# PlantandFoodResearch/MCHap

Hardware: AMD Instinct MI355X
Metric: loci/sec (whole node) for 1000-step MCMC, tetraploid 8-SNV loci, 1/2/4/8 GPUs (higher is better)
Workload: dtype f64; 1 GPU; 10000 synthetic tetraploid loci per GPU, 8 SNVs, 200 reads, 1000 MCMC steps x 2 chains, burn 500, posterior summary (BASELINE.json configs[1]); 4 passes in flight on separate HIP streams, each with its own device buffers; loci_per_gpu=10000, ploidy=4, snvs=8, reads=200, mcmc_steps=1000, chains=2, burn=500, llk_cache=True, passes_in_flight=4, hw_queues=4, world_size=1, devices=1

## Files before the change

### mchap_amd/csrc/denovo_simt_kernel.hpp

```cpp
#pragma once
#include "denovo_kernel.hpp"

namespace mchap {

constexpr int META_I_MH = 0;
constexpr int META_I_STATUS = 1;
constexpr int META_I_NDICT = 2;
constexpr int META_I_FLAT = 3;
constexpr int META_I_W01 = 4;
constexpr int META_I_COLS = 5;
__host__ __device__ inline int meta_i_stride(int max_pos) { return 5 + 2 * max_pos; }
constexpr uint16_t ND_W01 = 0x8000u;
__host__ __device__ inline int nd_count(uint16_t x) { return (int)(x & 0x7FFFu); }
__host__ __device__ inline bool nd_w01(uint16_t x) { return (x & ND_W01) != 0; }
constexpr int DICT_MAX = 128;
constexpr int DICT_HASH = 512;
__host__ __device__ inline int meta_f_prior(int) { return 1; }
__host__ __device__ inline int meta_f_dist(int max_ploidy) { return 1 + 2 * max_ploidy + 5; }
__host__ __device__ inline int meta_f_stride(int max_ploidy, int max_pos, int max_allele) {
  return 1 + 2 * max_ploidy + 5 + max_pos * max_allele;
}

struct SimtParams {
  DenovoParams d;
  double *rt;
  double *cntw;
  uint8_t *codes;
  double *dict;
  double *gbp;
  int32_t *meta_i;
  double *meta_f;
  int n_units;
  int max_pos, max_allele, max_ploidy;
  int max_ma;
  int max_ugens_pad;
  int prep_rows_off;
  int cstride;
  int flags;
  void *lane_state;
  void *lane_memo;
  void *pipe_state;
  double *pipe_memo;
  const int32_t *pipe_list;
  const int32_t *pipe_count;
  int32_t *pipe_out;
  int32_t *pipe_out_count;
  int pipe_iters;
  int pipe_iters_max;
  int pipe_mode;
  int pipe_parts;
  int bp_cache;
  int fill_lt, fill_kw;
  int tw_lds;
  int word_bits;
  uint64_t cache_epoch;
  uint64_t *ctx;
  int ctx_n;
};
constexpr int PIPE_RESUME = 1;
constexpr int PIPE_EXPORT = 2;
constexpr int PIPE_FILLONLY = 4;
constexpr int PIPE_NOFILL = 8;
constexpr int PIPE_FILL_SLOTS = 1024;
__host__ __device__ inline int pipe_parts_eff(int n_list, int parts) {
  if (parts <= 1 || n_list <= 0) return 1;
  const int pe = PIPE_FILL_SLOTS / n_list;
  return pe < 1 ? 1 : (pe > parts ? parts : pe);
}
struct PipeState {
  uint64_t g[8];
  double llk;
  uint64_t ctr;
  double mlo, mhi;
  int32_t step;
  int32_t mvalid;
  uint64_t pad[3];
};
static_assert(sizeof(PipeState) == 128, "PipeState layout");
constexpr int SIMT_FLAG_PREP_GLOBAL = 1 << 30;

#ifndef MCHAP_PREP_WPE
#define MCHAP_PREP_WPE 4
#endif
template <int RPL>
__global__ __launch_bounds__(64, MCHAP_PREP_WPE) void denovo_prepare_kernel(const SimtParams P) {
  extern __shared__ __align__(16) unsigned char smem[];
  const DenovoParams &D = P.d;
  const int u = blockIdx.x;
  const mchap_unit U = D.units[u];
  const int lane = threadIdx.x;
  const int R = U.n_reads, M0 = U.n_pos, A = U.max_allele, K = U.ploidy;
  const int rpad = D.rpad;
  const int MA = M0 * A;
  double *rt = P.rt + (size_t)u * P.max_ma * rpad;
  const bool in_lds = !(P.flags & SIMT_FLAG_PREP_GLOBAL);
  double *rl = in_lds ? reinterpret_cast<double *>(smem) : rt;
  double *lp = reinterpret_cast<double *>(smem) + (in_lds ? (size_t)MA * rpad : 0);
  const double *gr = D.reads ? D.reads + U.reads_off : nullptr;
  const int8_t *nal0 = D.n_alleles + U.nalleles_off;
  auto rawv = [&](int r, int q) -> double {
    if (gr) return gr[(size_t)r * MA + q];
    const int j = q / A, a = q - j * A;
    if (a >= nal0[j]) return 0.0;
    const size_t e = (size_t)U.reads_off + (size_t)r * M0 + j;
    const int call = D.calls[e];
    if (call < 0) return NAN;
    int qi = D.quals ? (int)D.quals[e] : 0;
    qi = qi < 0 ? 0 : (qi >= D.qual_prob_len ? D.qual_prob_len - 1 : qi);
    const double pc = D.qual_prob[qi];
    return a == call ? pc : (1.0 - pc) / 3.0;
  };
  double *cw = P.cntw + (size_t)u * rpad;
  int32_t *mi = P.meta_i + (size_t)u * meta_i_stride(P.max_pos);
  double *mf = P.meta_f + (size_t)u * meta_f_stride(P.max_ploidy, P.max_pos, P.max_allele);

  bool all_gaps = true;
  for (int r = lane; r < rpad; r += WAVE) {
    for (int q0 = 0; q0 < MA; q0 += 8) {
      double v[8];
#pragma unroll
      for (int k = 0; k < 8; k++) v[k] = (r < R && q0 + k < MA) ? rawv(r, q0 + k) : 1.0;
#pragma unroll
      for (int k = 0; k < 8; k++) {
        const int q = q0 + k;
        if (q < MA) {
          const double x = isnan(v[k]) ? 1.0 : v[k];
          if (in_lds) rl[(size_t)q * rpad + r] = x;
          rt[(size_t)q * rpad + r] = x;
          if (q % A < (int)nal0[q / A]) all_gaps = all_gaps && (x == 1.0);
        }
      }
    }
  }
  {
    const bool flat = __ballot(!all_gaps) == 0ull;
    if (lane == 0) mi[META_I_FLAT] = flat ? 1 : 0;
  }
  double cnt[RPL];
#pragma unroll
  for (int i = 0; i < RPL; i++) {
    const int r = lane + WAVE * i;
    cnt[i] = (r < R) ? (U.counts_off >= 0 ? (double)D.counts[U.counts_off + r] : 1.0) : 0.0;
    cw[r] = cnt[i];
  }
  {
    bool w01 = true;
#pragma unroll
    for (int i = 0; i < RPL; i++) w01 = w01 && (cnt[i] == 0.0 || cnt[i] == 1.0);
    const bool all01 = __ballot(!w01) == 0ull;
    if (lane == 0) mi[META_I_W01] = (all01 && !(P.flags & (1 << 20))) ? 1 : 0;
  }
  __syncthreads();
  {
    unsigned long long *hkeys = reinterpret_cast<unsigned long long *>(lp + P.max_ugens_pad);
    uint16_t *hcode = reinterpret_cast<uint16_t *>(hkeys + DICT_HASH);
    int *ndist = reinterpret_cast<int *>(hcode + DICT_HASH);
    const unsigned long long EMPTY = ~0ull;
    for (int i = lane; i < DICT_HASH; i += WAVE) hkeys[i] = EMPTY;
    if (lane == 0) *ndist = 0;
    __syncthreads();
    const int RPLT = rpad / WAVE;
    for (int q = 0; q < MA; q++) {
      for (int i0 = 0; i0 < RPL; i0 += 4) {
      unsigned long long keys[4];
#pragma unroll
      for (int k = 0; k < 4; k++) keys[k] = (unsigned long long)__double_as_longlong(rt[(size_t)q * rpad + lane + WAVE * min(i0 + k, RPL - 1)]);
#pragma unroll
      for (int k = 0; k < 4; k++) {
        if (i0 + k >= RPL) break;
        const unsigned long long key = keys[k];
        unsigned slot = (unsigned)(mix64(key) & (DICT_HASH - 1));
        while (*(volatile int *)ndist <= DICT_MAX) {
          unsigned long long old = *(volatile unsigned long long *)&hkeys[slot];
          if (old == EMPTY) {
            old = atomicCAS(&hkeys[slot], EMPTY, key);
            if (old == EMPTY) atomicAdd(ndist, 1);
          }
          if (old == EMPTY || old == key) break;
          slot = (slot + 1) & (DICT_HASH - 1);
        }
      }
      }
    }
    __syncthreads();
    const int nd = *ndist;
    uint8_t *ct = P.codes + (size_t)u * P.max_ma * WAVE * P.cstride;
    double *dict = P.dict + (size_t)u * DICT_MAX;
    if (nd <= DICT_MAX) {
      int base = 0;
      for (int s0 = 0; s0 < DICT_HASH; s0 += WAVE) {
        const unsigned long long key = hkeys[s0 + lane];
        const bool occ = key != EMPTY;
        const unsigned long long m = __ballot(occ);
        const int code = base + __popcll(m & ((1ull << lane) - 1ull));
        if (occ) {
          hcode[s0 + lane] = (uint16_t)code;
          dict[code] = __longlong_as_double((long long)key);
        }
        base += __popcll(m);
      }
      __syncthreads();
      for (int q = 0; q < MA; q++) {
        for (int i0 = 0; i0 < RPL; i0 += 4) {
          unsigned long long keys[4];
#pragma unroll
          for (int k = 0; k < 4; k++) keys[k] = (unsigned long long)__double_as_longlong(rt[(size_t)q * rpad + lane + WAVE * min(i0 + k, RPL - 1)]);
          uint32_t packed = 0;
#pragma unroll
          for (int k = 0; k < 4; k++) {
            if (i0 + k >= RPL) break;
            const unsigned long long key = keys[k];
            unsigned slot = (unsigned)(mix64(key) & (DICT_HASH - 1));
            while (hkeys[slot] != key) slot = (slot + 1) & (DICT_HASH - 1);
            if (RPL > 2) packed |= (uint32_t)(uint8_t)hcode[slot] << (8 * k);
            else ct[((size_t)q * WAVE + lane) * P.cstride + i0 + k] = (uint8_t)hcode[slot];
          }
          if (RPL > 2) *reinterpret_cast<uint32_t *>(ct + ((size_t)q * WAVE + lane) * P.cstride + i0) = packed;
        }
      }
    }
    if (lane == 0) mi[META_I_NDICT] = nd <= DICT_MAX ? nd : 0;
  }
  const int8_t *nalleles = D.n_alleles + U.nalleles_off;
  int Mh = 0;
  double luh = 0.0;
  const bool pow2_ploidy = (K & (K - 1)) == 0;
  const double inv_ploidy = 1.0 / (double)K;
  constexpr int KP = MCHAP_MAX_PLOIDY_DENOVO;
  __shared__ double s_lg1[KP + 1];
  __shared__ double s_lga[(MCHAP_MAX_ALLELE + 1) * (KP + 1)];
  __shared__ double s_lgb[MCHAP_MAX_ALLELE + 1], s_left[MCHAP_MAX_ALLELE + 1];
  const double Fp = U.inbreeding;
  const bool with_prior = !isnan(Fp);
  if (with_prior) {
    for (int d = lane; d <= K; d += WAVE) s_lg1[d] = lgamma((double)d + 1.0);
    if (Fp != 0.0) {
      for (int e = lane; e < (A + 1) * (K + 1); e += WAVE) {
        const int n = e / (K + 1), d = e % (K + 1);
        if (n >= 1 && d >= 1) s_lga[n * (KP + 1) + d] = lgamma((double)d + (1.0 / (double)n) * ((1.0 - Fp) / Fp));
      }
      for (int n = 1 + lane; n <= A; n += WAVE) {
        const double alpha = (1.0 / (double)n) * ((1.0 - Fp) / Fp);
        const double sum_alphas = alpha * (double)n;
        s_lgb[n] = lgamma(alpha);
        s_left[n] = (lgamma((double)K + 1.0) + lgamma(sum_alphas)) - lgamma((double)K + sum_alphas);
      }
    }
    __syncthreads();
  }
  auto snv_prior = [&](uint64_t g, int n) -> double {
    int dose[KP];
    for (int i = 0; i < K; i++) dose[i] = 0;
    for (int i = 0; i < K; i++) {
      int j = 0;
      while (nib(g, i) != nib(g, j)) j++;
      dose[j] += 1;
    }
    if (Fp == 0.0) {
      double den = 0.0;
      for (int i = 0; i < K; i++) den += s_lg1[dose[i]];
      return (s_lg1[K] - den) - (double)K * c_ln[n];
    }
    double prod = 0.0;
    for (int i = 0; i < K; i++)
      if (dose[i] > 0) prod += s_lga[n * (KP + 1) + dose[i]] - (s_lg1[dose[i]] + s_lgb[n]);
    return s_left[n] + prod;
  };
  double *pl = reinterpret_cast<double *>(smem + P.prep_rows_off);
  for (int j = 0; j < M0; j++) {
    const int n = nalleles[j];
    const int u_gens = snv_genotypes(n, K);
    const double *rowp = rl + (size_t)(j * A) * rpad;
    if (!in_lds) {
      for (int a = 0; a < A; a++)
#pragma unroll
        for (int i = 0; i < RPL; i++) pl[(size_t)a * rpad + lane + WAVE * i] = rt[(size_t)(j * A + a) * rpad + lane + WAVE * i];
      rowp = pl;
    }
    uint64_t g = 0;
    for (int q = 0; q < u_gens; q++) {
      double lprior = 0.0;
      if (with_prior) lprior = snv_prior(g, n);
      double s = 0.0;
#pragma unroll
      for (int i = 0; i < RPL; i++) {
        double rp = 0.0;
        if (pow2_ploidy) {
          for (int h = 0; h < K; h++) rp += rowp[(size_t)nib(g, h) * rpad + lane + WAVE * i] * inv_ploidy;
        } else {
          for (int h = 0; h < K; h++) rp += rowp[(size_t)nib(g, h) * rpad + lane + WAVE * i] / (double)K;
        }
        s += read_log(rp) * cnt[i];
      }
      const double llk = wave_sum(s);
      lp[q] = lprior + llk;
      g = increment_snv_genotype(g, K);
    }
    double acc = lp[0];
    for (int q = 1; q < u_gens; q++) acc = add_log_prob(acc, lp[q]);
    int fixed_allele = -1;
    for (int a = 0; a < n; a++) {
      int idx = 0;
      for (int i = 0; i < K; i++) idx += (a == 0) ? 0 : snv_genotypes(a, i + 1);
      if (exp(lp[idx] - acc) >= D.fix_hom) fixed_allele = a;
    }
    if (lane == 0) D.fixed[U.fixed_off + j] = (int8_t)fixed_allele;
    if (fixed_allele < 0) {
      if (lane == 0) {
        mi[META_I_COLS + Mh] = j * A;
        mi[META_I_COLS + P.max_pos + Mh] = n;
      }
      luh += c_ln[n];
      Mh++;
    }
  }
  const int bits = allele_bits(A);
  int status = MCHAP_UNIT_OK;
  if (Mh == 0) status = MCHAP_UNIT_ALL_FIXED;
  else if (Mh * bits > (P.word_bits ? P.word_bits : 64)) status = MCHAP_ERR_LIMIT;
  else if (U.initial_off >= 0 && U.initial_n_het != Mh) status = MCHAP_UNIT_BAD_INITIAL;
  if (lane == 0) {
    mi[META_I_MH] = Mh;
    mi[META_I_STATUS] = status;
    D.status[u] = status;
    mf[0] = luh;
  }
  if (status != MCHAP_UNIT_OK) {
    if (status == MCHAP_UNIT_ALL_FIXED) {
      const size_t tb = U.trace_off, lb = U.llk_off;
      const int S = D.steps, C_ = D.chains;
      for (int i = lane; i < C_ * S * K; i += WAVE) D.trace[tb + i] = 0ull;
      for (int i = lane; i < C_ * S; i += WAVE) D.llks[lb + i] = NAN;
    }
    return;
  }
  if (!isnan(U.inbreeding) && lane == 0) {
    double *t = mf + meta_f_prior(0);
    const double F = U.inbreeding;
    for (int d = 0; d <= K; d++) t[K + 1 + d] = lgamma((double)d + 1.0);
    t[2 * K + 3] = lgamma((double)K + 1.0);
    t[2 * K + 4] = (double)K * luh;
    if (F != 0.0) {
      const double log_disp = log((1.0 - F) / F) - luh;
      const double disp = exp(log_disp);
      const double sum_disp = exp(log_disp + luh);
      const double lg_disp = lgamma(disp);
      t[0] = 0.0;
      for (int d = 1; d <= K; d++) t[d] = lgamma((double)d + disp) - (lgamma((double)d + 1.0) + lg_disp);
      t[2 * K + 2] = (lgamma((double)K + 1.0) + lgamma(sum_disp)) - lgamma((double)K + sum_disp);
    }
  }
  if (U.initial_off < 0) {
    double *dist = mf + meta_f_dist(P.max_ploidy);
    __syncthreads();
    for (int jj = 0; jj < Mh; jj++) {
      const int col = mi[META_I_COLS + jj];
      int n_nonzero = 0;
      uint32_t gapmask = 0;
      double dv[MCHAP_MAX_ALLELE];
      for (int a = 0; a < A; a++) {
        double tot = 0.0;
        int n_ok = 0, n_nz = 0;
        for (int i0 = 0; i0 < RPL; i0 += 4) {
          double v4[4];
#pragma unroll
          for (int k = 0; k < 4; k++) {
            const int r = lane + WAVE * (i0 + k);
            v4[k] = (i0 + k < RPL && r < R) ? rawv(r, col + a) : 0.0;
          }
#pragma unroll
          for (int k = 0; k < 4; k++) {
            const int r = lane + WAVE * (i0 + k);
            if (i0 + k < RPL && r < R) {
              const double v = v4[k];
              if (!isnan(v)) {
                tot += v;
                n_ok++;
              }
              if (!(v == 0.0)) n_nz++;
            }
          }
        }
        tot = wave_sum(tot);
        n_ok = wave_sum_i(n_ok);
        n_nz = wave_sum_i(n_nz);
        if (n_ok == 0) {
          gapmask |= 1u << a;
          dv[a] = 1.0;
          n_nonzero++;
        } else {
          dv[a] = tot / (double)n_ok;
          if (n_nz > 0) n_nonzero++;
        }
      }
      for (int a = 0; a < A; a++)
        if (gapmask & (1u << a)) dv[a] = 1.0 / (double)n_nonzero;
      double s = 0.0;
      for (int a = 1; a < A; a++) s += dv[a];
      s = (A > 1) ? dv[0] + s : dv[0];
      if (lane == 0)
        for (int a = 0; a < A; a++) dist[jj * A + a] = dv[a] / s;
    }
  }
}

typedef unsigned __int128 u128;
template <class W> struct WordBits { static constexpr int value = 8 * (int)sizeof(W); };
__device__ __forceinline__ int word_popc(uint64_t x) { return __popcll(x); }
__device__ __forceinline__ int word_popc(u128 x) { return __popcll((uint64_t)x) + __popcll((uint64_t)(x >> 64)); }
__device__ __forceinline__ int word_ffs(uint64_t x) { return __ffsll((long long)x); }
__device__ __forceinline__ int word_ffs(u128 x) {
  const uint64_t lo = (uint64_t)x, hi = (uint64_t)(x >> 64);
  return lo ? __ffsll((long long)lo) : (hi ? 64 + __ffsll((long long)hi) : 0);
}
__device__ __forceinline__ uint64_t word_mix(uint64_t t, uint64_t x) { return mix64(t ^ x) + 0x9E3779B97F4A7C15ull; }
__device__ __forceinline__ uint64_t word_mix(uint64_t t, u128 x) {
  t = mix64(t ^ (uint64_t)(x >> 64)) + 0x9E3779B97F4A7C15ull;
  return mix64(t ^ (uint64_t)x) + 0x9E3779B97F4A7C15ull;
}

template <class W> struct PackOf { typedef uint32_t type; static constexpr int KMAX = MCHAP_MAX_PLOIDY; };
template <> struct PackOf<u128> { typedef uint64_t type; static constexpr int KMAX = MCHAP_MAX_PLOIDY_DENOVO; };

template <class W>
struct SimtLdsT {
  W *w;
  W *pw;
  double *llk_t;
  uint64_t *rngn;
  double *prior;
  uint8_t *optin;
  uint16_t *sub;
  uint16_t *cols;
  uint8_t *shift;
  uint8_t *nal;
};
typedef SimtLdsT<uint64_t> SimtLds;

__host__ __device__ inline size_t simt_lds_bytes(int Kmax, int Mmax, int T, int word_bytes = 8) {
  size_t b = 0;
  b += (size_t)word_bytes * T * Kmax * 64;
  b += (size_t)word_bytes * Kmax * 64;
  b += (size_t)8 * T * 64 * 2;
  b += (size_t)8 * (2 * Kmax + 5) * 64;
  b += (size_t)Kmax * Kmax * 64;
  b += (size_t)2 * Kmax * Mmax * 64;
  b += (size_t)2 * Mmax * 64;
  b += (size_t)1 * Mmax * 64 * 2;
  return (b + 15) & ~(size_t)15;
}

// ... 737 lines not shown
```

### mchap_amd/csrc/mchap_hip.hip

```cpp
#include <hip/hip_runtime.h>

#include <cmath>
#include <cstdarg>
#include <cstdio>
#include <cstdlib>
#include <cstring>
#include <algorithm>
#include <atomic>
#include <mutex>
#include <vector>

#include "../../include/mchap_hip.h"
#include "denovo_kernel.hpp"
#include "denovo_simt_kernel.hpp"
#include "denovo_spec_kernel.hpp"
#include "denovo_fillw_kernel.hpp"
#ifdef MCHAP_TEST_KERNELS
#include "denovo_fill_kernel.hpp"
#include "denovo_lane_kernel.hpp"
#endif
#include "exact_kernel.hpp"
#include "call_mcmc_kernel.hpp"
#include "posterior_kernel.hpp"

// ... 182 lines not shown
}

struct DevBuf {
  void *p = nullptr;
  ~DevBuf() {
    if (p) (void)hipFree(p);
  }
  template <class T>
  T *as() const { return reinterpret_cast<T *>(p); }
};

struct HostCall {
  hipStream_t stream = nullptr;
  int open() {
    HIP_TRY(hipStreamCreateWithFlags(&stream, hipStreamNonBlocking));
    return MCHAP_OK;
  }
  ~HostCall() {
    if (stream) (void)hipStreamDestroy(stream);
  }
  int up(void *dst, const void *src, size_t bytes) {
    HIP_TRY(hipMemcpyAsync(dst, src, bytes, hipMemcpyHostToDevice, stream));
    return MCHAP_OK;
  }
  int down(void *dst, const void *src, size_t bytes) {
    HIP_TRY(hipMemcpyAsync(dst, src, bytes, hipMemcpyDeviceToHost, stream));
    return MCHAP_OK;
  }
  int sync() {
    HIP_TRY(hipStreamSynchronize(stream));
    return MCHAP_OK;
  }
};
#define MCHAP_TRY(expr)       \
  do {                        \
    const int rc_ = (expr);   \
    if (rc_) return rc_;      \
  } while (0)

size_t up256(size_t x) { return (x + 255) & ~(size_t)255; }
struct DevArena {
  DevBuf buf;
  size_t cap = 0, off = 0;
  int reserve(size_t bytes) {
    cap = bytes + 4096;
    if (hipMalloc(&buf.p, cap) != hipSuccess) return fail(MCHAP_ERR_HIP, "hipMalloc of %zu bytes", cap);
    return MCHAP_OK;
  }
  template <class T>
  T *take(size_t n) {
    T *p = reinterpret_cast<T *>(reinterpret_cast<unsigned char *>(buf.p) + off);
    off += up256(n * sizeof(T));
    return off <= cap ? p : nullptr;
  }
};

int code_stride(int rpl) { return rpl <= 2 ? rpl : (rpl + 3) & ~3; }

int rpl_for(int max_reads) {
  const int need = (max_reads + 63) / 64;
  for (int r : {1, 2, 4, 8, 16})
    if (need <= r) return r;
  return -1;
}

int validate_cfg(const mchap_denovo_cfg *cfg) {
  if (!cfg) return fail(MCHAP_ERR_BAD_ARG, "cfg is NULL");
  if (cfg->steps < 1 || cfg->chains < 1) return fail(MCHAP_ERR_BAD_ARG, "steps and chains must be >= 1");
  if (cfg->chains > 65535) return fail(MCHAP_ERR_LIMIT, "chains > 65535");
  if (cfg->n_temps < 1 || cfg->n_temps > MCHAP_MAX_TEMPS) return fail(MCHAP_ERR_LIMIT, "n_temps out of range");
  for (int t = 1; t < cfg->n_temps; t++)
    if (cfg->temperatures[t] < cfg->temperatures[t - 1]) return fail(MCHAP_ERR_BAD_ARG, "temperatures must be ascending");
  if (cfg->temperatures[0] < 0.0) return fail(MCHAP_ERR_BAD_ARG, "temperatures must be >= 0");
  if (cfg->temperatures[cfg->n_temps - 1] != 1.0) return fail(MCHAP_ERR_BAD_ARG, "last temperature must be 1.0");
  if (cfg->n_intervals == 0 && !cfg->break_table) return fail(MCHAP_ERR_BAD_ARG, "break_table required when n_intervals is None");
#ifndef MCHAP_TEST_KERNELS
  if (cfg->kernel == 1 || cfg->kernel == 4)
    return fail(MCHAP_ERR_BAD_ARG, "kernel %d is only built into libmchap_hip_test.so (make test-kernels)", cfg->kernel);
#endif
  if (cfg->kernel < 0 || cfg->kernel > 5) return fail(MCHAP_ERR_BAD_ARG, "kernel %d: not one of 0..5", cfg->kernel);
  return MCHAP_OK;
}

struct Tune {
  int cache_slots = 1024, flags = 0, spec_group = 0, pipe_first = 0, pipe_resume = 8, pipe_rounds = 2, pipe_max = 64, pipe_parts = 8;
  int pipe_group = 64;
  size_t prep_lds_limit = 8 * 1024;
  int pipe_stop = 0;
  bool cache_auto = true;
};
Tune tune_of(const mchap_denovo_cfg *cfg) {
  Tune t;
  const mchap_denovo_tuning *u = cfg->tuning;
  if (!u) return t;
  if (u->cache_slots >= 64 && u->cache_slots <= 65536 && (u->cache_slots & (u->cache_slots - 1)) == 0) {
    t.cache_slots = u->cache_slots;
    t.cache_auto = false;
  }
  t.flags = u->flags;
  if (u->spec_group == 16 || u->spec_group == 32 || u->spec_group == 64) t.spec_group = u->spec_group;
  if (u->pipe_first > 0) t.pipe_first = u->pipe_first;
  if (u->pipe_resume > 0) t.pipe_resume = u->pipe_resume;
  if (u->pipe_rounds > 0) t.pipe_rounds = u->pipe_rounds - 1;
  if (u->pipe_max > 0) t.pipe_max = u->pipe_max;
  if (u->pipe_parts > 0 && u->pipe_parts <= 64) t.pipe_parts = u->pipe_parts;
  if (u->prep_lds_limit > 0) t.prep_lds_limit = (size_t)u->prep_lds_limit;
  t.pipe_stop = u->pipe_stop;
#ifdef MCHAP_TEST_KERNELS
  if (u->reserved[0] == 16 || u->reserved[0] == 32) t.pipe_group = u->reserved[0];
#endif
  return t;
}

size_t break_table_bytes(const mchap_denovo_cfg *cfg) {
  const size_t mp = cfg->max_pos > 0 ? (size_t)cfg->max_pos : 1;
  return ((mp + 1) * mp * sizeof(double) + 255) & ~(size_t)255;
}

struct BatchDims {
  int max_reads = 1, max_pos = 1, max_allele = 1, max_ploidy = 1, max_ma = 1, max_ugens = 1;
  int min_reads = 1 << 30;
  int uniform_ploidy = -1;
};

bool use_simt(const mchap_denovo_cfg *cfg);
int batch_dims(const mchap_denovo_cfg *cfg, int n_units, const mchap_unit *units_host, BatchDims &B) {
  for (int u = 0; u < n_units; u++) {
    const mchap_unit &U = units_host[u];
    const int kmax = use_simt(cfg) ? MCHAP_MAX_PLOIDY_DENOVO : MCHAP_MAX_PLOIDY;
    if (U.ploidy < 1 || U.ploidy > kmax) return fail(MCHAP_ERR_LIMIT, "unit %d: ploidy %d not in 1..%d", u, U.ploidy, kmax);
    if (U.max_allele < 1 || U.max_allele > MCHAP_MAX_ALLELE) return fail(MCHAP_ERR_LIMIT, "unit %d: max_allele %d not in 1..%d", u, U.max_allele, MCHAP_MAX_ALLELE);
    if (U.n_reads < 1 || U.n_reads > MCHAP_MAX_READS) return fail(MCHAP_ERR_LIMIT, "unit %d: n_reads %d not in 1..%d (zero reads are mocked by the caller as one NaN read)", u, U.n_reads, MCHAP_MAX_READS);
    if (U.n_pos < 1 || U.n_pos > MCHAP_MAX_POS) return fail(MCHAP_ERR_LIMIT, "unit %d: n_pos %d not in 1..%d", u, U.n_pos, MCHAP_MAX_POS);
    if (cfg->n_intervals == 0 && U.n_pos > cfg->max_pos) return fail(MCHAP_ERR_BAD_ARG, "unit %d: n_pos exceeds break_table", u);
    B.max_reads = std::max(B.max_reads, U.n_reads);
    B.min_reads = std::min(B.min_reads, U.n_reads);
    B.max_pos = std::max(B.max_pos, U.n_pos);
    B.max_allele = std::max(B.max_allele, U.max_allele);
    B.max_ploidy = std::max(B.max_ploidy, U.ploidy);
    B.uniform_ploidy = (B.uniform_ploidy < 0 || B.uniform_ploidy == U.ploidy) ? U.ploidy : 0;
    B.max_ma = std::max(B.max_ma, U.n_pos * U.max_allele);
    B.max_ugens = std::max(B.max_ugens, mchap::snv_genotypes(U.max_allele, U.ploidy));
  }
  return MCHAP_OK;
}

int spec_group(const Tune &T, int K, int max_pos) {
  if (K < 2 || K > 8) return 0;
  const int n = K * max_pos;
  int g = T.spec_group ? T.spec_group : 16;
  while (g < 64 && (g < K * (K - 1) || 2 * g < n)) g *= 2;
  const int slots = (g == 64) ? 3 : 2;
  if (g < K * (K - 1) || slots * g < n) return 0;
  if ((K == 5 || K == 6) && g < 32) g = 32;
  if (K >= 7) g = 64;
  return g;
}

bool lane_supported(int K, int max_pos, int n_temps) {
#ifdef MCHAP_TEST_KERNELS
  if (n_temps != 1 || K < 1 || K > 8) return false;
  const int slots = (K == 8) ? 3 : 2;
  return K * max_pos <= slots * 64 && K * (K - 1) <= 64;
#else
  return false;
#endif
// ... 639 lines not shown
  P.seed = cfg->seed;
  P.rpad = rpad;
  P.max_pos = cfg->max_pos > 0 ? cfg->max_pos : 1;
  {
    const size_t n = (size_t)(P.max_pos + 1) * P.max_pos;
    const size_t bt_bytes = break_table_bytes(cfg);
    if (!workspace || workspace_bytes < (int64_t)bt_bytes)
      return fail(MCHAP_ERR_BAD_ARG, "workspace of %lld bytes is too small (mchap_denovo_workspace_bytes)", (long long)workspace_bytes);
    double *bt_dev = reinterpret_cast<double *>(workspace);
    if (cfg->break_table)
      HIP_TRY(hipMemcpyAsync(bt_dev, cfg->break_table, n * sizeof(double), hipMemcpyHostToDevice, stream));
    else
      HIP_TRY(hipMemsetAsync(bt_dev, 0, n * sizeof(double), stream));
    P.break_table = bt_dev;
    workspace = reinterpret_cast<unsigned char *>(workspace) + bt_bytes;
    workspace_bytes -= (int64_t)bt_bytes;
  }
  HIP_TRY(hipMemsetAsync(status, 0, sizeof(int32_t) * n_units, stream));
  P.cache = nullptr;
  P.cache_slots = 0;

  if (use_simt(cfg)) {
    const int want_slots = cache_slots_of(cfg, T, pl, n_units, B);
    int slots = want_slots;
    SimtCarve cv = simt_carve(cfg, pl, n_units, B, rpad, slots);
    while (slots >= 32 && (int64_t)cv.total > workspace_bytes) {
      slots >>= 1;
      cv = simt_carve(cfg, pl, n_units, B, rpad, slots);
    }
    if (slots < 32 && want_slots) {
      slots = 0;
      cv = simt_carve(cfg, pl, n_units, B, rpad, 0);
    }
    if (!workspace || (int64_t)cv.total > workspace_bytes)
      return fail(MCHAP_ERR_BAD_ARG, "workspace of %lld bytes is too small: kernel %d needs at least %zu (mchap_denovo_workspace_bytes)",
                  (long long)workspace_bytes, cfg->kernel, cv.total);
    unsigned char *ws = reinterpret_cast<unsigned char *>(workspace);
    if (ctx_shape(pl, B, T) && workspace_bytes > (int64_t)cv.total) {
      const int cn = ctx_slots_for((size_t)(workspace_bytes - (int64_t)cv.total), (size_t)n_units * cfg->chains, ctx_slot_bytes(pl, B));
      if (cn > 0) {
        SP.ctx = reinterpret_cast<uint64_t *>(ws + cv.ctx);
        SP.ctx_n = cn;
      }
    }
    if (slots > 0) {
      P.cache = reinterpret_cast<uint64_t *>(ws + cv.cache);
      P.cache_slots = slots;
      uint64_t epoch = 0;
      if ((pl.kind == SAMPLER_PIPE || pl.kind == SAMPLER_SPEC) && !(T.flags & (64 | 65536)) &&
          B.max_ploidy * mchap::allele_bits(B.max_allele) * B.max_pos <= 32) {
        epoch = cfg->cache_epoch > 0 ? (uint64_t)cfg->cache_epoch : g_cache_epoch.fetch_add(1) + 1;
        if (epoch >= (1ull << 31) - 1) epoch = 0;
      }
      SP.cache_epoch = epoch << 33;
      if (!epoch)
        HIP_TRY(hipMemsetAsync(ws + cv.cache, 0, (size_t)n_units * cfg->chains * (pl.kind == SAMPLER_SPEC ? cfg->n_temps : 1) * slots * 16, stream));
      if (cv.key_words) {
        P.cache_keys = reinterpret_cast<uint64_t *>(ws + cv.ckeys);
        P.cache_key_words = cv.key_words;
      }
    }
    SP.rt = reinterpret_cast<double *>(ws + cv.rt);
    SP.cntw = reinterpret_cast<double *>(ws + cv.cntw);
    SP.codes = ws + cv.codes;
    SP.dict = reinterpret_cast<double *>(ws + cv.dict);
    SP.gbp = (cv.has_gbp && !(T.flags & 512)) ? reinterpret_cast<double *>(ws + cv.gbp) : nullptr;
    SP.meta_i = reinterpret_cast<int32_t *>(ws + cv.meta_i);
    SP.meta_f = reinterpret_cast<double *>(ws + cv.meta_f);
    SP.lane_state = ws + cv.lane_state;
    SP.lane_memo = ws + cv.lane_memo;
    SP.pipe_state = ws + cv.pipe_state;
    SP.pipe_memo = reinterpret_cast<double *>(ws + cv.pipe_memo);
    SP.n_units = n_units;
    SP.max_pos = B.max_pos;
    SP.max_allele = B.max_allele;
    SP.max_ploidy = B.max_ploidy;
    SP.max_ma = B.max_ma;
    SP.cstride = code_stride(rpl);
    SP.flags = T.flags & (63 | 128 | 2048 | 4096 | 262144 | (1 << 20));
    SP.max_ugens_pad = (B.max_ugens + 8) & ~7;
    const size_t lds_dict = (size_t)mchap::DICT_HASH * (8 + 2) + 64;
    size_t lds_prep = (size_t)B.max_ma * rpad * 8 + (size_t)SP.max_ugens_pad * 8 + lds_dict;
    SP.prep_rows_off = 0;
    if (lds_prep > 160 * 1024 || (size_t)B.max_ma * rpad * 8 > T.prep_lds_limit) {
      lds_prep = (size_t)SP.max_ugens_pad * 8 + lds_dict;
      lds_prep = (lds_prep + 15) & ~(size_t)15;
      SP.prep_rows_off = (int)lds_prep;
      lds_prep += (size_t)B.max_allele * rpad * 8;
      SP.flags |= mchap::SIMT_FLAG_PREP_GLOBAL;
    }
    const size_t lds_simt = mchap::simt_lds_bytes(B.max_ploidy, B.max_pos, cfg->n_temps, pl.wide ? 16 : 8);
    SP.word_bits = pl.wide ? 128 : 64;
    if (lds_prep > 160 * 1024 || lds_simt > 160 * 1024)
      return fail(MCHAP_ERR_LIMIT, "a unit needs %zu / %zu bytes of LDS (> 160 KiB)", lds_prep, lds_simt);
    auto prepare = [&](const mchap::SimtParams &Q, int n, hipStream_t st) {
      switch (rpl) {
        case 1: return launch_prepare<1>(Q, n, lds_prep, st);
        case 2: return launch_prepare<2>(Q, n, lds_prep, st);
        case 3: return launch_prepare<3>(Q, n, lds_prep, st);
        case 4: return launch_prepare<4>(Q, n, lds_prep, st);
        case 5: return launch_prepare<5>(Q, n, lds_prep, st);
        case 6: return launch_prepare<6>(Q, n, lds_prep, st);
        case 7: return launch_prepare<7>(Q, n, lds_prep, st);
        case 8: return launch_prepare<8>(Q, n, lds_prep, st);
        case 12: return launch_prepare<12>(Q, n, lds_prep, st);
        case 16: return launch_prepare<16>(Q, n, lds_prep, st);
        case 24: return launch_prepare<24>(Q, n, lds_prep, st);
        case 32: return launch_prepare<32>(Q, n, lds_prep, st);
        case 48: return launch_prepare<48>(Q, n, lds_prep, st);
        default: return launch_prepare<64>(Q, n, lds_prep, st);
      }
    };
    rc = prepare(SP, n_units, stream);
    if (rc) return rc;
    switch (pl.kind) {
#ifdef MCHAP_TEST_KERNELS
      case SAMPLER_LANE: return launch_lane(T, pl.K, SP, n_units, cfg->chains, cfg->timer, stream);
#endif
      case SAMPLER_PIPE:
        return launch_pipe(T, pl.K, pl.G, SP, n_units, cfg->chains, reinterpret_cast<int32_t *>(ws + cv.pipe_lists),
                           reinterpret_cast<int32_t *>(ws + cv.pipe_counts), cfg->timer, stream, B.min_reads <= 64, B.max_reads);
      case SAMPLER_SPEC: return launch_spec(T, pl.K, pl.G, SP, n_units, cfg->chains, cfg->n_temps, cfg->timer, stream);
      default: return launch_simt(pl.K, SP, n_units, cfg->chains, lds_simt, cfg->timer, stream, pl.wide);
    }
  }

#ifdef MCHAP_TEST_KERNELS
  size_t lds = 0;
  for (int u = 0; u < n_units; u++) {
    const mchap_unit &U = units_host[u];
    const mchap::WaveLayout L = mchap::wave_layout(U.ploidy, U.n_pos, U.max_allele, cfg->n_temps);
    const int cpb = cfg->chains < mchap::CHAINS_PER_BLOCK ? cfg->chains : mchap::CHAINS_PER_BLOCK;
    const size_t need = (size_t)U.n_pos * U.max_allele * rpad * 8 + (size_t)cpb * L.total;
    if (need > lds) lds = need;
  }
  if (lds > 160 * 1024)
    return fail(MCHAP_ERR_LIMIT, "a unit needs %zu bytes of LDS (> 160 KiB): dense float64 staging does not fit", lds);
  if (cfg->llk_cache && workspace && workspace_bytes > 0) {
    const int64_t rows = (int64_t)n_units * cfg->chains;
    int slots = T.cache_slots;
    while (slots >= 16 && rows * slots * 16 > workspace_bytes) slots >>= 1;
    if (slots >= 16) {
      P.cache = reinterpret_cast<uint64_t *>(workspace);
      P.cache_slots = slots;
      HIP_TRY(hipMemsetAsync(workspace, 0, (size_t)(rows * slots * 16), stream));
    }
  }
  return launch_denovo(rpl, P, n_units, cfg->chains, lds, cfg->timer, stream);
#else
  return fail(MCHAP_ERR_BAD_ARG, "kernel 1 is only built into libmchap_hip_test.so");
#endif
}

int mchap_denovo_fit_batch(const mchap_denovo_cfg *cfg, int n_units, const mchap_unit *units, const double *reads,
                           int64_t reads_len, const int64_t *read_counts, int64_t counts_len, const int8_t *n_alleles,
                           int64_t nalleles_len, const int8_t *initial, int64_t initial_len, uint64_t *trace_words,
                           int64_t trace_len, double *llks, int64_t llks_len, int8_t *fixed_alleles, int64_t fixed_len,
                           int32_t *status) {
  int rc = validate_cfg(cfg);
  if (rc) return rc;
  rc = ensure_init();
  if (rc) return rc;
  if (n_units <= 0) return MCHAP_OK;
  DevBuf d_units, d_reads, d_counts, d_nal, d_init, d_trace, d_llk, d_fixed, d_status, d_ws;
  const int64_t ws_bytes = mchap_denovo_workspace_bytes(cfg, n_units, units);
  if (ws_bytes < 0) return fail(MCHAP_ERR_LIMIT, "unsupported unit shape");
  HostCall hc;
// ... 158 lines not shown
```

Measured before the change: 1.176 million loci/s.

## Build the read dictionary in one pass and keep prep rows as LDS byte codes

Adds a single-pass prepare mode. While the reads are first loaded, each value is hashed into a smaller LDS dictionary and an 8-bit slot index is stored per read, plus per-wave gap bitmasks. Later stages (SNV genotype likelihoods, code emission, column stats) then work from the LDS slot codes and dictionary instead of re-reading the global read table or recomputing the raw values. For pipe/spec samplers the global read-table writes are skipped unless the dictionary overflows, which trims global traffic in the prepare kernel at the cost of extra LDS, atomics during loading and added code complexity.

```diff
diff --git a/mchap_amd/csrc/denovo_simt_kernel.hpp b/mchap_amd/csrc/denovo_simt_kernel.hpp
--- a/mchap_amd/csrc/denovo_simt_kernel.hpp
+++ b/mchap_amd/csrc/denovo_simt_kernel.hpp
@@ -78,6 +78,15 @@
 };
 static_assert(sizeof(PipeState) == 128, "PipeState layout");
 constexpr int SIMT_FLAG_PREP_GLOBAL = 1 << 30;
+constexpr int SIMT_FLAG_PREP_ONCE = 1 << 29;
+constexpr int SIMT_FLAG_PREP_ROWS = 1 << 28;
+constexpr int DICT_HASH_ONCE = 256;
+__host__ __device__ inline int prep_slot_stride(int rpl) { return (rpl + 3) & ~3; }
+__host__ __device__ inline size_t prep_once_bytes(int max_ma, int max_allele, int rpl) {
+  const size_t t = (size_t)max_ma * rpl * 8 + (size_t)max_ma * 64 * prep_slot_stride(rpl);
+  const size_t rows = (size_t)max_allele * 64 * rpl * 8;
+  return t > rows ? t : rows;
+}
 
 #ifndef MCHAP_PREP_WPE
 #define MCHAP_PREP_WPE 4
@@ -94,6 +103,8 @@
   const int MA = M0 * A;
   double *rt = P.rt + (size_t)u * P.max_ma * rpad;
   const bool in_lds = !(P.flags & SIMT_FLAG_PREP_GLOBAL);
+  const bool once = (P.flags & SIMT_FLAG_PREP_ONCE) != 0;
+  const bool rows_always = !once || (P.flags & SIMT_FLAG_PREP_ROWS) != 0;
   double *rl = in_lds ? reinterpret_cast<double *>(smem) : rt;
   double *lp = reinterpret_cast<double *>(smem) + (in_lds ? (size_t)MA * rpad : 0);
   const double *gr = D.reads ? D.reads + U.reads_off : nullptr;
@@ -113,6 +124,32 @@
   double *cw = P.cntw + (size_t)u * rpad;
   int32_t *mi = P.meta_i + (size_t)u * meta_i_stride(P.max_pos);
   double *mf = P.meta_f + (size_t)u * meta_f_stride(P.max_ploidy, P.max_pos, P.max_allele);
+  const int HS = once ? DICT_HASH_ONCE : DICT_HASH;
+  unsigned long long *hkeys = reinterpret_cast<unsigned long long *>(lp + P.max_ugens_pad);
+  uint16_t *hcode = reinterpret_cast<uint16_t *>(hkeys + HS);
+  int *ndist = reinterpret_cast<int *>(hcode + HS);
+  const unsigned long long EMPTY = ~0ull;
+  constexpr int SST = (RPL + 3) & ~3;
+  unsigned long long *gapm = reinterpret_cast<unsigned long long *>(smem + P.prep_rows_off);
+  uint8_t *sl = reinterpret_cast<uint8_t *>(gapm + (size_t)P.max_ma * RPL);
+  if (once) {
+    for (int i = lane; i < HS; i += WAVE) hkeys[i] = EMPTY;
+    if (lane == 0) *ndist = 0;
+    __syncthreads();
+  }
+  auto slot_of = [&](unsigned long long key) -> unsigned {
+    unsigned slot = (unsigned)(mix64(key) & (DICT_HASH_ONCE - 1));
+    while (*(volatile int *)ndist <= DICT_MAX) {
+      unsigned long long old = *(volatile unsigned long long *)&hkeys[slot];
+      if (old == EMPTY) {
+        old = atomicCAS(&hkeys[slot], EMPTY, key);
+        if (old == EMPTY) atomicAdd(ndist, 1);
+      }
+      if (old == EMPTY || old == key) break;
+      slot = (slot + 1) & (DICT_HASH_ONCE - 1);
+    }
+    return slot;
+  };
 
   bool all_gaps = true;
   for (int r = lane; r < rpad; r += WAVE) {
@@ -126,8 +163,13 @@
         if (q < MA) {
           const double x = isnan(v[k]) ? 1.0 : v[k];
           if (in_lds) rl[(size_t)q * rpad + r] = x;
-          rt[(size_t)q * rpad + r] = x;
+          if (rows_always) rt[(size_t)q * rpad + r] = x;
           if (q % A < (int)nal0[q / A]) all_gaps = all_gaps && (x == 1.0);
+          if (once) {
+            const unsigned long long gm = __ballot(isnan(v[k]));
+            if (lane == 0) gapm[q * RPL + r / WAVE] = gm;
+            sl[(q * WAVE + lane) * SST + r / WAVE] = (uint8_t)slot_of((unsigned long long)__double_as_longlong(x));
+          }
         }
       }
     }
@@ -151,11 +193,54 @@
     if (lane == 0) mi[META_I_W01] = (all01 && !(P.flags & (1 << 20))) ? 1 : 0;
   }
   __syncthreads();
-  {
-    unsigned long long *hkeys = reinterpret_cast<unsigned long long *>(lp + P.max_ugens_pad);
-    uint16_t *hcode = reinterpret_cast<uint16_t *>(hkeys + DICT_HASH);
-    int *ndist = reinterpret_cast<int *>(hcode + DICT_HASH);
-    const unsigned long long EMPTY = ~0ull;
+  bool from_lds = false;
+  if (once) {
+    const int nd = *ndist;
+    uint8_t *ct = P.codes + (size_t)u * P.max_ma * WAVE * P.cstride;
+    double *dict = P.dict + (size_t)u * DICT_MAX;
+    if (nd <= DICT_MAX) {
+      from_lds = true;
+      int base = 0;
+      for (int s0 = 0; s0 < DICT_HASH_ONCE; s0 += WAVE) {
+        const unsigned long long key = hkeys[s0 + lane];
+        const bool occ = key != EMPTY;
+        const unsigned long long m = __ballot(occ);
+        const int code = base + __popcll(m & ((1ull << lane) - 1ull));
+        if (occ) {
+          hcode[s0 + lane] = (uint16_t)code;
+          dict[code] = __longlong_as_double((long long)key);
+        }
+        base += __popcll(m);
+      }
+      __syncthreads();
+      for (int q = 0; q < MA; q++) {
+        for (int i0 = 0; i0 < RPL; i0 += 4) {
+          const uint32_t w = *reinterpret_cast<const uint32_t *>(sl + (q * WAVE + lane) * SST + i0);
+          uint32_t packed = 0;
+#pragma unroll
+          for (int k = 0; k < 4; k++) {
+            if (i0 + k >= RPL) break;
+            const uint8_t code = (uint8_t)hcode[(w >> (8 * k)) & 0xFFu];
+            if (RPL > 2) packed |= (uint32_t)code << (8 * k);
+            else ct[((size_t)q * WAVE + lane) * P.cstride + i0 + k] = code;
+          }
+          if (RPL > 2) *reinterpret_cast<uint32_t *>(ct + ((size_t)q * WAVE + lane) * P.cstride + i0) = packed;
+        }
+      }
+    } else if (!rows_always) {
+      for (int r = lane; r < rpad; r += WAVE) {
+        for (int q0 = 0; q0 < MA; q0 += 8) {
+          double v[8];
+#pragma unroll
+          for (int k = 0; k < 8; k++) v[k] = (r < R && q0 + k < MA) ? rawv(r, q0 + k) : 1.0;
+#pragma unroll
+          for (int k = 0; k < 8; k++)
+            if (q0 + k < MA) rt[(size_t)(q0 + k) * rpad + r] = isnan(v[k]) ? 1.0 : v[k];
+        }
+      }
+    }
+    if (lane == 0) mi[META_I_NDICT] = nd <= DICT_MAX ? nd : 0;
+  } else {
     for (int i = lane; i < DICT_HASH; i += WAVE) hkeys[i] = EMPTY;
     if (lane == 0) *ndist = 0;
     __syncthreads();
@@ -271,7 +356,7 @@
     const int n = nalleles[j];
     const int u_gens = snv_genotypes(n, K);
     const double *rowp = rl + (size_t)(j * A) * rpad;
-    if (!in_lds) {
+    if (!in_lds && !from_lds) {
       for (int a = 0; a < A; a++)
 #pragma unroll
         for (int i = 0; i < RPL; i++) pl[(size_t)a * rpad + lane + WAVE * i] = rt[(size_t)(j * A + a) * rpad + lane + WAVE * i];
@@ -282,15 +367,35 @@
       double lprior = 0.0;
       if (with_prior) lprior = snv_prior(g, n);
       double s = 0.0;
-#pragma unroll
-      for (int i = 0; i < RPL; i++) {
-        double rp = 0.0;
-        if (pow2_ploidy) {
-          for (int h = 0; h < K; h++) rp += rowp[(size_t)nib(g, h) * rpad + lane + WAVE * i] * inv_ploidy;
-        } else {
-          for (int h = 0; h < K; h++) rp += rowp[(size_t)nib(g, h) * rpad + lane + WAVE * i] / (double)K;
-        }
-        s += read_log(rp) * cnt[i];
+      if (from_lds) {
+#pragma unroll
+        for (int i0 = 0; i0 < RPL; i0 += 4) {
+          double rp4[4] = {0.0, 0.0, 0.0, 0.0};
+          for (int h = 0; h < K; h++) {
+            const uint32_t w = *reinterpret_cast<const uint32_t *>(sl + ((j * A + (int)nib(g, h)) * WAVE + lane) * SST + i0);
+#pragma unroll
+            for (int k = 0; k < 4; k++) {
+              if (i0 + k >= RPL) break;
+              const double x = __longlong_as_double((long long)hkeys[(w >> (8 * k)) & 0xFFu]);
+              if (pow2_ploidy) rp4[k] += x * inv_ploidy;
+              else rp4[k] += x / (double)K;
+            }
+          }
+#pragma unroll
+          for (int k = 0; k < 4; k++)
+            if (i0 + k < RPL) s += read_log(rp4[k]) * cnt[i0 + k];
+        }
+      } else {
+#pragma unroll
+        for (int i = 0; i < RPL; i++) {
+          double rp = 0.0;
+          if (pow2_ploidy) {
+            for (int h = 0; h < K; h++) rp += rowp[(size_t)nib(g, h) * rpad + lane + WAVE * i] * inv_ploidy;
+          } else {
+            for (int h = 0; h < K; h++) rp += rowp[(size_t)nib(g, h) * rpad + lane + WAVE * i] / (double)K;
+          }
+          s += read_log(rp) * cnt[i];
+        }
       }
       const double llk = wave_sum(s);
       lp[q] = lprior + llk;
@@ -363,10 +468,21 @@
         int n_ok = 0, n_nz = 0;
         for (int i0 = 0; i0 < RPL; i0 += 4) {
           double v4[4];
-#pragma unroll
-          for (int k = 0; k < 4; k++) {
-            const int r = lane + WAVE * (i0 + k);
-            v4[k] = (i0 + k < RPL && r < R) ? rawv(r, col + a) : 0.0;
+          if (from_lds) {
+            const uint32_t w = *reinterpret_cast<const uint32_t *>(sl + ((col + a) * WAVE + lane) * SST + i0);
+#pragma unroll
+            for (int k = 0; k < 4; k++) {
+              const int r = lane + WAVE * (i0 + k);
+              v4[k] = 0.0;
+              if (i0 + k < RPL && r < R)
+                v4[k] = ((gapm[(col + a) * RPL + i0 + k] >> lane) & 1ull) ? NAN : __longlong_as_double((long long)hkeys[(w >> (8 * k)) & 0xFFu]);
+            }
+          } else {
+#pragma unroll
+            for (int k = 0; k < 4; k++) {
+              const int r = lane + WAVE * (i0 + k);
+              v4[k] = (i0 + k < RPL && r < R) ? rawv(r, col + a) : 0.0;
+            }
           }
 #pragma unroll
           for (int k = 0; k < 4; k++) {
diff --git a/mchap_amd/csrc/mchap_hip.hip b/mchap_amd/csrc/mchap_hip.hip
--- a/mchap_amd/csrc/mchap_hip.hip
+++ b/mchap_amd/csrc/mchap_hip.hip
@@ -288,6 +288,7 @@
   return MCHAP_OK;
 }
 
+constexpr size_t PREP_ONCE_LDS = 16 * 1024;
 struct Tune {
   int cache_slots = 1024, flags = 0, spec_group = 0, pipe_first = 0, pipe_resume = 8, pipe_rounds = 2, pipe_max = 64, pipe_parts = 8;
   int pipe_group = 64;
@@ -1093,7 +1094,15 @@
     const size_t lds_dict = (size_t)mchap::DICT_HASH * (8 + 2) + 64;
     size_t lds_prep = (size_t)B.max_ma * rpad * 8 + (size_t)SP.max_ugens_pad * 8 + lds_dict;
     SP.prep_rows_off = 0;
-    if (lds_prep > 160 * 1024 || (size_t)B.max_ma * rpad * 8 > T.prep_lds_limit) {
+    const size_t once_bytes = mchap::prep_once_bytes(B.max_ma, B.max_allele, rpl);
+    if (!(T.flags & 2097152) && once_bytes <= PREP_ONCE_LDS) {
+      const size_t lds_dict_once = (size_t)mchap::DICT_HASH_ONCE * (8 + 2) + 64;
+      lds_prep = ((size_t)SP.max_ugens_pad * 8 + lds_dict_once + 15) & ~(size_t)15;
+      SP.prep_rows_off = (int)lds_prep;
+      lds_prep += once_bytes;
+      SP.flags |= mchap::SIMT_FLAG_PREP_GLOBAL | mchap::SIMT_FLAG_PREP_ONCE;
+      if (!(pl.kind == SAMPLER_PIPE || pl.kind == SAMPLER_SPEC) || (T.flags & (4 | 64))) SP.flags |= mchap::SIMT_FLAG_PREP_ROWS;
+    } else if (lds_prep > 160 * 1024 || (size_t)B.max_ma * rpad * 8 > T.prep_lds_limit) {
       lds_prep = (size_t)SP.max_ugens_pad * 8 + lds_dict;
       lds_prep = (lds_prep + 15) & ~(size_t)15;
       SP.prep_rows_off = (int)lds_prep;
```

Measured after the change: 1.135 million loci/s. 3.5% lower.
